# TzuYaoHuang/WaterLily.jl

Measured on AMD Instinct MI355X. Metric: cells*steps/sec (3D TGV) ; smoother HBM GB/s vs peak, higher is better.
Workload: dtype f32; 1 GPU; 3D Taylor-Green vortex 512^3 Float32, wall-bounded, Re=1600, NoBody, remeasure=false (BASELINE configs[4] domain on 1 GPU); size=512, resjac=630, resjac_redo=0

## Files before the change

waterlily.jl_amd/csrc/wl_convf.hip:

```cpp
#include <cstdlib>
#include <type_traits>

#include "wl_bcfold.hpp"
#include "wl_conv_cell.hpp"

namespace {
#define CF_TX 32
#define CF_TY 16
#define CF_N (CF_TX * CF_TY)
#define CF_CX (2 * CF_TX)
#define CF_CY CF_TY
#define CF_W (CF_CX + 4)
#define CF_H (CF_CY + 4)
#define CF_P (CF_W * CF_H)
#define CF_SLOT (3 * CF_P)
#define CF_NSLOT 3
#define CF_HPC (CF_P / 2 - CF_CX / 2 * CF_CY)
#define CF_FYC ((CF_CY + 1) * CF_CX)
#define CF_FY (3 * CF_FYC)
#define CF_FX (3 * CF_CY)
#define CF_FBUF (CF_FY + CF_FX)
#define CF_NGEN (3 * CF_CX + 3 * CF_CY)
#define CF_LDS (CF_NSLOT * CF_SLOT + 2 * CF_FBUF)

struct __attribute__((aligned(4))) F2v { float x, y; };
__device__ __forceinline__ float2 cf_ldg2(const float* __restrict__ p, unsigned o) { const F2v t = *reinterpret_cast<const F2v*>(p + o); return make_float2(t.x, t.y); }
__device__ __forceinline__ void cf_stg2(float* __restrict__ p, unsigned o, float2 v) { F2v t; t.x = v.x; t.y = v.y; *reinterpret_cast<F2v*>(p + o) = t; }
__device__ __forceinline__ float2 cf_lds2(const float* p) { return *reinterpret_cast<const float2*>(p); }
__device__ __forceinline__ float cf_sel(const float2& v, int e) { return e ? v.y : v.x; }
__device__ __forceinline__ float cf_next_lane(float v) {
  return __int_as_float(__builtin_amdgcn_update_dpp(__float_as_int(v), __float_as_int(v), 0x130 , 0xf, 0xf, false));
}

struct CfPair { unsigned off; int mode; };
__device__ __forceinline__ CfPair cf_pair_addr(int X, int Y, int nx, int ny, unsigned sy) {
  CfPair r;
  const int Yc = Y < 0 ? 0 : (Y > ny - 1 ? ny - 1 : Y);
  int Xc = X, mode = 0;
  if (X < 0) { Xc = X + 1; mode = 1; }
  else if (X + 1 > nx - 1) { Xc = X - 1; mode = 2; }
  if (Xc < 0 || Xc + 1 > nx - 1 || Y != Yc) { mode = 3; Xc = Xc < 0 ? 0 : (Xc + 1 > nx - 1 ? nx - 2 : Xc); }
  r.off = (unsigned)Xc + (unsigned)Yc * sy; r.mode = mode;
  return r;
}
__device__ __forceinline__ float2 cf_pair_fix(float2 t, int mode) { return make_float2(mode == 2 ? t.y : t.x, mode == 1 ? t.x : t.y); }

template <int SCH, int WALLS>
__device__ __forceinline__ float cf_flux(float U, float a, float b, float c, float d, bool wl, bool wu, float nu) {
  const bool pos = U > 0;
  float X = lam<SCH>(pos ? a : d, pos ? b : c, pos ? c : b);
  if (WALLS) {
    const bool use_avg = (wl && pos) || (wu && (U < 0));
    X = use_avg ? (c + b) / 2 : X;
  }
  return U * X - nu * (c - b);
}

int g_convf_on = 1;

template <int SCH, int FULL, int U0ADV, int MODE, int PROJ>
__global__ void __launch_bounds__(CF_N, 4) k_conv_flux(GridX g, const float* __restrict__ u, float nu, int ka, int kb, int zchunk, BdimArgs bd) {
  __shared__ float lds[CF_LDS];
  const int ntx = (g.nx - 2 + CF_CX - 1) / CF_CX, nty = (g.ny - 2 + CF_CY - 1) / CF_CY;
  const int ntiles = ntx * nty;
  const unsigned h = blockIdx.x, q = h & 7u, s = h >> 3;
  const unsigned per = (unsigned)((ntiles + 7) >> 3);
  const int c = (int)(s / per);
  const int tl = (int)(q * per + (s - (unsigned)c * per));
  if (tl >= ntiles) return;
  const int ks = ka + c * zchunk, ke = (ks + zchunk < kb) ? ks + zchunk : kb;
  if (ks >= ke) return;
  const int tx = tl % ntx, ty = tl / ntx;
  const int x0 = 1 + tx * CF_CX, y0 = 1 + ty * CF_CY;
  const int tid = threadIdx.x, lx = tid & (CF_TX - 1), ly = tid >> 5;
  const int x = x0 + 2 * lx, y = y0 + ly;
  const int my = (ly + 2) * CF_W + 2 + 2 * lx;
  const bool in0 = FULL || (y <= g.ny - 2 && x <= g.nx - 2), in1 = FULL || (y <= g.ny - 2 && x + 1 <= g.nx - 2);
  const unsigned cs = (unsigned)g.cs, sz = (unsigned)g.sz, sy = (unsigned)g.sy;
  CfPair pc;
  if (FULL) { pc.off = (unsigned)x + (unsigned)y * sy; pc.mode = 0; } else pc = cf_pair_addr(x, y, g.nx, g.ny, sy);
  const int hid = tid < 3 * CF_HPC ? tid : 3 * CF_HPC - 1;
  const int hcmp = hid / CF_HPC, hh = hid - hcmp * CF_HPC;
  int R, col;
  if (hh < 4 * (CF_W / 2)) { const int rr = hh / (CF_W / 2); const int m = hh - rr * (CF_W / 2); R = rr < 2 ? rr : rr + CF_CY; col = 2 * m; }
  else { const int h2 = hh - 4 * (CF_W / 2); R = 2 + (h2 >> 1); col = (h2 & 1) ? CF_W - 2 : 0; }
  const CfPair ph = cf_pair_addr(x0 - 2 + col, y0 - 2 + R, g.nx, g.ny, sy);
  const unsigned hbase = (unsigned)hcmp * cs + ph.off;
  const int hl = hcmp * CF_P + R * CF_W + col;
  const bool gen = tid < CF_NGEN;
  int ga, gF, gsb, gb, gout; bool gwu;
  if (tid < 3 * CF_CX) { ga = tid >> 6; const int gj = tid & 63; gF = (2 + CF_CY) * CF_W + 2 + gj; gsb = CF_W; gb = 1; gwu = (y0 + CF_CY == g.ny - 1); gout = ga * CF_FYC + CF_CY * CF_CX + gj; }
  else { const int t = (tid - 3 * CF_CX) & 63; ga = t >> 4; const int gr = t & 15; gF = (2 + gr) * CF_W + 2 + CF_CX; gsb = 1; gb = 0; gwu = (x0 + CF_CX == g.nx - 1); gout = CF_FY + (ga > 2 ? 2 : ga) * CF_CY + gr; }
  if (ga > 2) ga = 2;
  const int gf = ga * CF_P + gF;
  const int gU0 = gb * CF_P + gF;
  const int gUm = gU0 - (ga == 0 ? 1 : CF_W);
  for (int i = tid; i < CF_LDS; i += CF_N) lds[i] = 0.f;
  __syncthreads();

  struct Stage { float2 c[3]; float2 h; };
  unsigned ho[2] = {0u, 0u}, hnb = 0u; bool hd[2] = {false, false}; float hU = 0.f, hc = 0.f;
  const float* __restrict__ px = bd.px;
  if (PROJ) {
#pragma unroll
    for (int e = 0; e < 2; e++) {
      const int Xe = x0 - 2 + col + e, Ye = y0 - 2 + R;
      const int Xc = Xe < 1 ? 1 : (Xe > g.nx - 2 ? g.nx - 2 : Xe), Yc = Ye < 1 ? 1 : (Ye > g.ny - 2 ? g.ny - 2 : Ye);
      ho[e] = (unsigned)Xc + (unsigned)Yc * sy;
      hd[e] = hcmp == 0 ? (Xe <= 1 || Xe >= g.nx - 1) : (hcmp == 1 ? (Ye <= 1 || Ye >= g.ny - 1) : false);
    }
    hnb = hcmp == 0 ? 1u : (hcmp == 1 ? sy : sz);
    hU = hcmp == 0 ? bd.bcU[0] : (hcmp == 1 ? bd.bcU[1] : bd.bcU[2]);
    hc = hcmp == 0 ? bd.cl_c[0] : (hcmp == 1 ? bd.cl_c[1] : bd.cl_c[2]);
  }
  auto load_plane = [&](int kk) -> Stage {
    const int kc = PROJ ? (kk < 1 ? 1 : (kk > g.nz - 2 ? g.nz - 2 : kk)) : (kk < 0 ? 0 : (kk > g.nz - 1 ? g.nz - 1 : kk));
    const unsigned ko = (unsigned)kc * sz;
    Stage st;
#pragma unroll
    for (int cc = 0; cc < 3; cc++) st.c[cc] = cf_ldg2(u, (unsigned)cc * cs + ko + pc.off);
    if (PROJ) { st.h.x = u[(unsigned)hcmp * cs + ko + ho[0]]; st.h.y = u[(unsigned)hcmp * cs + ko + ho[1]]; }
    else st.h = cf_ldg2(u, hbase + ko);
    return st;
  };
  struct XStage { float2 xc, xy, xk; float xm; float xh[2], xn[2]; };
  auto load_x = [&](int kk) -> XStage {
    const int kc = kk < 1 ? 1 : (kk > g.nz - 2 ? g.nz - 2 : kk);
    const unsigned ko = (unsigned)kc * sz;
    XStage X;
    X.xc = cf_ldg2(px, ko + pc.off); X.xm = px[ko + pc.off - 1u]; X.xy = cf_ldg2(px, ko + pc.off - sy); X.xk = cf_ldg2(px, ko - sz + pc.off);
#pragma unroll
    for (int e = 0; e < 2; e++) { X.xh[e] = px[ko + ho[e]]; X.xn[e] = px[ko + ho[e] - hnb]; }
    return X;
  };
  const bool dxc0 = (x == 1), dyc = (y == 1);
  auto project = [&](Stage& st, const XStage& X, int kk) {
    const bool zd = kk <= 1 || kk >= g.nz - 1;
    const float c0 = bd.cl_c[0], c1 = bd.cl_c[1], c2 = bd.cl_c[2];
    const float p0x = st.c[0].x - c0 * (X.xc.x - X.xm), p0y = st.c[0].y - c0 * (X.xc.y - X.xc.x);
    const float p1x = st.c[1].x - c1 * (X.xc.x - X.xy.x), p1y = st.c[1].y - c1 * (X.xc.y - X.xy.y);
    const float p2x = st.c[2].x - c2 * (X.xc.x - X.xk.x), p2y = st.c[2].y - c2 * (X.xc.y - X.xk.y);
    st.c[0] = make_float2(dxc0 ? bd.bcU[0] : p0x, p0y);
    st.c[1] = make_float2(dyc ? bd.bcU[1] : p1x, dyc ? bd.bcU[1] : p1y);
    st.c[2] = make_float2(zd ? bd.bcU[2] : p2x, zd ? bd.bcU[2] : p2y);
    const float h0 = st.h.x - hc * (X.xh[0] - X.xn[0]), h1 = st.h.y - hc * (X.xh[1] - X.xn[1]);
    const bool hz = hcmp == 2 && zd;
    st.h = make_float2((hd[0] || hz) ? hU : h0, (hd[1] || hz) ? hU : h1);
  };
  auto slot_of = [&](int kk) -> float* { return lds + ((unsigned)(kk + 3) % 3u) * CF_SLOT; };
  auto write_plane = [&](int kk, const Stage& st) {
    float* sl = slot_of(kk);
#pragma unroll
    for (int cc = 0; cc < 3; cc++) *reinterpret_cast<float2*>(sl + cc * CF_P + my) = FULL ? st.c[cc] : cf_pair_fix(st.c[cc], pc.mode);
    *reinterpret_cast<float2*>(sl + hl) = PROJ ? st.h : cf_pair_fix(st.h, ph.mode);
  };
  const bool wlx = (x == 1);
  const bool wux0 = (x == g.nx - 1), wux1 = (x + 1 == g.nx - 1);
  const bool wly = (y == 1), wuy0 = (y == g.ny - 1);
  float zf[3][2];
  float2 Zm1[3];
  float gprev = 0.f;

  auto zfaces = [&](auto ztag, int k, const float2* Zm, const float2* C1, const float2* Zp1, const float2* Zp2, const float* Pp, float (*Pz)[2]) {
    const int Kg = g.gk + k;
    const bool wlz = (Kg + 1 == 1), wuz = (Kg + 1 == g.gnz - 1);
    const float2 Exz = cf_lds2(Pp + 2 * CF_P - 2);
    const float2 Eyz = cf_lds2(Pp + 2 * CF_P - CF_W);
#pragma unroll
    for (int a = 0; a < 3; a++) {
#pragma unroll
      for (int e = 0; e < 2; e++) {
        float Uz;
        if (a == 0) Uz = (cf_sel(Zp1[2], e) + (e ? Zp1[2].x : Exz.y)) / 2;
        else if (a == 1) Uz = (cf_sel(Zp1[2], e) + cf_sel(Eyz, e)) / 2;
        else Uz = (cf_sel(Zp1[2], e) + cf_sel(C1[2], e)) / 2;
        Pz[a][e] = cf_flux<SCH, decltype(ztag)::value>(Uz, cf_sel(Zm[a], e), cf_sel(C1[a], e), cf_sel(Zp1[a], e), cf_sel(Zp2[a], e), wlz, wuz, nu);
      }
    }
  };
  Stage S; XStage XS;
  {
    float2 m2[3];
    if (PROJ) { Stage sm = load_plane(ks - 2); const XStage xm = load_x(ks - 2); project(sm, xm, ks - 2); for (int cc = 0; cc < 3; cc++) m2[cc] = sm.c[cc]; }
    else {
      const unsigned ko = (unsigned)(ks - 2 < 0 ? 0 : ks - 2) * sz;
#pragma unroll
      for (int cc = 0; cc < 3; cc++) { m2[cc] = cf_ldg2(u, (unsigned)cc * cs + ko + pc.off); if (!FULL) m2[cc] = cf_pair_fix(m2[cc], pc.mode); }
    }
    Stage s0 = load_plane(ks - 1), s1 = load_plane(ks), s2 = load_plane(ks + 1);
    if (PROJ) {
      const XStage x0s = load_x(ks - 1), x1s = load_x(ks), x2s = load_x(ks + 1);
      project(s0, x0s, ks - 1); project(s1, x1s, ks); project(s2, x2s, ks + 1);
    }
    S = load_plane(ks + 2);
    if (PROJ) XS = load_x(ks + 2);
    write_plane(ks - 1, s0); write_plane(ks, s1); write_plane(ks + 1, s2);
    float2 C1[3], Zp1[3], Zp2[3];
#pragma unroll
    for (int cc = 0; cc < 3; cc++) {
      C1[cc] = FULL ? s0.c[cc] : cf_pair_fix(s0.c[cc], pc.mode); Zp1[cc] = FULL ? s1.c[cc] : cf_pair_fix(s1.c[cc], pc.mode); Zp2[cc] = FULL ? s2.c[cc] : cf_pair_fix(s2.c[cc], pc.mode);
    }
    __syncthreads();
    zfaces(std::integral_constant<int, 1>{}, ks - 1, m2, C1, Zp1, Zp2, slot_of(ks) + my, zf);
    if (gen) gprev = slot_of(ks - 1)[gU0];
#pragma unroll
    for (int cc = 0; cc < 3; cc++) Zm1[cc] = C1[cc];
    __syncthreads();
  }
  const float dtv = bd.dt_dev ? *bd.dt_dev : bd.dt;
  const int N[3] = {g.nx, g.ny, g.gnz};
  const float mw[2][2] = {{wl::wl_cl_coef(x + 1, N[0], bd.cl_c[0]), wl::wl_cl_coef(x + 2, N[0], bd.cl_c[0])}, {wl::wl_cl_coef(y + 1, N[1], bd.cl_c[1]), wl::wl_cl_coef(y + 1, N[1], bd.cl_c[1])}};
  const bool tile_walls = tx == 0 || tx == ntx - 1 || ty == 0 || ty == nty - 1;
  float2 un[3];
  auto store_plane = [&](auto wtag, int kq) {
    const unsigned kqo = (unsigned)kq * sz;
    if (decltype(wtag)::value && SCH != WL_VANLEER && bd.bc_on && (x <= 1 || x + 1 >= g.nx - 2 || y <= 1 || y >= g.ny - 2)) {
      if (in0) { const float v[3] = {un[0].x, un[1].x, un[2].x}; wl_bc_fold_store_xy(bd.uout, g, x, y, kq, v, bd.bcU); }
      if (in1) { const float v[3] = {un[0].y, un[1].y, un[2].y}; wl_bc_fold_store_xy(bd.uout, g, x + 1, y, kq, v, bd.bcU); }
      return;
    }
#pragma unroll
    for (int a = 0; a < 3; a++) {
      const unsigned oa = (unsigned)a * cs + kqo + pc.off;
      if (FULL) cf_stg2(bd.uout, oa, un[a]);
      else if (pc.mode == 0 && in0 && in1) cf_stg2(bd.uout, oa, un[a]);
      else { const unsigned o0 = (unsigned)a * cs + kqo + (unsigned)x + (unsigned)y * sy; if (in0) bd.uout[o0] = un[a].x; if (in1) bd.uout[o0 + 1] = un[a].y; }
    }
  };
  auto mainloop = [&](auto wtag) {
    constexpr int WALLS = decltype(wtag)::value;
    for (int k = ks; k < ke; k++) {
      if (PROJ) project(S, XS, k + 2);
      float2 Zp2[3];
#pragma unroll
      for (int cc = 0; cc < 3; cc++) Zp2[cc] = FULL ? S.c[cc] : cf_pair_fix(S.c[cc], pc.mode);
      write_plane(k + 2, S);
      S = load_plane(k + 3);
      const unsigned ko = (unsigned)k * sz;
      float2 u0v[3];
      if (k > ks) store_plane(wtag, k - 1);
      const float* S0 = slot_of(k);
      const float* P0 = S0 + my;
      const float* Pp = slot_of(k + 1) + my;
      float* FB = lds + CF_NSLOT * CF_SLOT + (k & 1) * CF_FBUF;
      float2 C1[3], Zp1[3];
#pragma unroll
      for (int cc = 0; cc < 3; cc++) { C1[cc] = cf_lds2(P0 + cc * CF_P); Zp1[cc] = cf_lds2(Pp + cc * CF_P); }
      float a0[3], a1[3], Pl1[3], Px0[3];
      {
        float2 CA[3], Ym2[3], Ym1[3], Yp1[3]; float CCx[3];
#pragma unroll
        for (int cc = 0; cc < 3; cc++) {
          CA[cc] = cf_lds2(P0 + cc * CF_P - 2); CCx[cc] = P0[cc * CF_P + 2];
          Ym2[cc] = cf_lds2(P0 + cc * CF_P - 2 * CF_W); Ym1[cc] = cf_lds2(P0 + cc * CF_P - CF_W); Yp1[cc] = cf_lds2(P0 + cc * CF_P + CF_W);
        }
        const float rx[4] = {CA[0].x, CA[0].y, C1[0].x, C1[0].y};
        const float ry[4] = {CA[1].x, CA[1].y, C1[1].x, C1[1].y};
#pragma unroll
        for (int a = 0; a < 3; a++) {
          const float r[5] = {CA[a].x, CA[a].y, C1[a].x, C1[a].y, CCx[a]};
          float Ux[2];
          if (a == 0) { Ux[0] = (rx[2] + rx[1]) / 2; Ux[1] = (rx[3] + rx[2]) / 2; }
          else if (a == 1) { Ux[0] = (rx[2] + Ym1[0].x) / 2; Ux[1] = (rx[3] + Ym1[0].y) / 2; }
          else { Ux[0] = (rx[2] + Zm1[0].x) / 2; Ux[1] = (rx[3] + Zm1[0].y) / 2; }
          const float PxA = cf_flux<SCH, WALLS>(Ux[0], r[0], r[1], r[2], r[3], wlx, wux0, nu);
          const float PxB = cf_flux<SCH, WALLS>(Ux[1], r[1], r[2], r[3], r[4], false, wux1, nu);
          float t0 = 0.f, t1 = 0.f;
          t0 = t0 + PxA; t0 = t0 - PxB;
          t1 = t1 + PxB;
          Px0[a] = PxA;
          float Pl[2];
#pragma unroll
          for (int e = 0; e < 2; e++) {
            const float vm2 = cf_sel(Ym2[a], e), vm1 = cf_sel(Ym1[a], e), v0 = cf_sel(C1[a], e), vp1 = cf_sel(Yp1[a], e);
            float Ul;
            if (a == 0) Ul = (ry[2 + e] + ry[1 + e]) / 2;
            else if (a == 1) Ul = (v0 + vm1) / 2;
            else Ul = (cf_sel(C1[1], e) + cf_sel(Zm1[1], e)) / 2;
            Pl[e] = cf_flux<SCH, WALLS>(Ul, vm2, vm1, v0, vp1, wly, wuy0, nu);
          }
          t0 = t0 + Pl[0];
          a0[a] = t0; a1[a] = t1; Pl1[a] = Pl[1];
          *reinterpret_cast<float2*>(FB + a * CF_FYC + ly * CF_CX + 2 * lx) = make_float2(Pl[0], Pl[1]);
        }
      }
      if (gen) {
        const float fa = S0[gf - 2 * gsb], fb = S0[gf - gsb], fc = S0[gf], fd = S0[gf + gsb];
        const float ub0 = S0[gU0], ubm = S0[gUm];
        const float U = (ub0 + (ga == 2 ? gprev : ubm)) / 2;
        gprev = ub0;
        FB[gout] = cf_flux<SCH, WALLS>(U, fa, fb, fc, fd, false, gwu, nu);
      }
      float Pz[3][2];
      const int Kg = g.gk + k;
      const bool zwall = (Kg + 1 == 1 || Kg + 1 == g.gnz - 1);
      if (zwall) zfaces(std::integral_constant<int, 1>{}, k, Zm1, C1, Zp1, Zp2, Pp, Pz);
      else zfaces(std::integral_constant<int, 0>{}, k, Zm1, C1, Zp1, Zp2, Pp, Pz);
      if (!U0ADV) {
#pragma unroll
        for (int a = 0; a < 3; a++) { u0v[a] = cf_ldg2(bd.u0, (unsigned)a * cs + ko + pc.off); if (!FULL) u0v[a] = cf_pair_fix(u0v[a], pc.mode); }
      }
      if (PROJ) XS = load_x(k + 3);
      __syncthreads();
      float2 PuA[3]; float PxE[3];
#pragma unroll
      for (int a = 0; a < 3; a++) {
        PuA[a] = cf_lds2(FB + a * CF_FYC + (ly + 1) * CF_CX + 2 * lx);
        PxE[a] = 0.f;
        if (lx == CF_TX - 1) PxE[a] = FB[CF_FY + a * CF_CY + ly];
      }
      const float mz = wl::wl_cl_coef(Kg + 1, N[2], bd.cl_c[2]);
#pragma unroll
      for (int a = 0; a < 3; a++) {
        float Px2 = cf_next_lane(Px0[a]);
        if (lx == CF_TX - 1) Px2 = PxE[a];
        const float2 Pu = PuA[a];
        float t0 = a0[a], t1 = a1[a];
        t0 = t0 - Pu.x;
        t1 = t1 - Px2; t1 = t1 + Pl1[a]; t1 = t1 - Pu.y;
        t0 = t0 + zf[a][0]; t0 = t0 - Pz[a][0]; zf[a][0] = Pz[a][0];
        t1 = t1 + zf[a][1]; t1 = t1 - Pz[a][1]; zf[a][1] = Pz[a][1];
        const float acc[2] = {t0, t1};
        const float2 u0a = U0ADV ? C1[a] : u0v[a];
        const float m00 = a == 2 ? mz : (WALLS ? mw[a][0] : bd.cl_c[a]), m01 = a == 2 ? mz : (WALLS ? mw[a][1] : bd.cl_c[a]);
#pragma unroll
        for (int e = 0; e < 2; e++) {
          const float fn = cf_sel(u0a, e) + dtv * acc[e] - 0.f;
          const float xx = (0.f / 2 + 0.f) + (e ? m01 : m00) * fn;
          float v;
          if (MODE == 1) v = xx;
          else if (MODE == 2) v = (cf_sel(C1[a], e) * bd.pre + xx) * bd.post;
          else { v = (bd.pre == 0.f) ? xx : (cf_sel(C1[a], e) * bd.pre + xx); if (bd.scale_after) v = v * bd.post; }
          if (e) un[a].y = v; else un[a].x = v;
        }
        Zm1[a] = C1[a];
      }
    }
    store_plane(wtag, ke - 1);
  };
  if (tile_walls) mainloop(std::integral_constant<int, 1>{}); else mainloop(std::integral_constant<int, 0>{});
}
}

namespace wl {
void conv_flux_enable(int on) { g_convf_on = on; }
bool conv_flux_on() { return g_convf_on != 0; }
bool conv_proj_ok(const GridX& g, unsigned per) {
  return g_convf_on && g.D == 3 && g.nz == g.gnz && g.k0 == 1 && g.k1 == g.nz - 1 && g.nz >= 6 && (g.nx - 2) % CF_CX == 0 && (g.ny - 2) % CF_CY == 0 && conv_tile_ok(g, per, g.k1 - g.k0);
}
int conv_flux(const float* u_adv, const GridX& g, float nu, int scheme, int ka, int kb, int zc, const void* bdp, hipStream_t s) {
  const BdimArgs bd = *(const BdimArgs*)bdp;
  const int ntiles = ((g.nx - 2 + CF_CX - 1) / CF_CX) * ((g.ny - 2 + CF_CY - 1) / CF_CY);
  const int per = (ntiles + 7) >> 3;
  const int np = kb - ka;
  const int nch = (np + zc - 1) / zc;
  const dim3 grid((unsigned)(8 * per * nch), 1, 1);
  const bool full = (g.nx - 2) % CF_CX == 0 && (g.ny - 2) % CF_CY == 0;
  const bool u0adv = bd.u0 == u_adv;
  const int mode = (u0adv && bd.pre == 0.f && !bd.scale_after) ? 1 : ((!u0adv && bd.pre != 0.f && bd.scale_after) ? 2 : 0);
  if (bd.px && !(full && mode == 2 && g.nz == g.gnz && ka == 1 && kb == g.nz - 1)) { wl_set_error("conv_flux: the fused projection needs whole tiles, the corrector's BDIM! form and the whole single domain"); return WL_EINVAL; }
#define WL_CF(SCHV, FULLV, ADV, MD, PJ) hipLaunchKernelGGL((k_conv_flux<SCHV, FULLV, ADV, MD, PJ>), grid, dim3(CF_N), 0, s, g, u_adv, nu, ka, kb, zc, bd)
#define WL_CF1(SCHV, FULLV) do { if (mode == 1) WL_CF(SCHV, FULLV, 1, 1, 0); else if (mode == 2) WL_CF(SCHV, FULLV, 0, 2, 0); else if (u0adv) WL_CF(SCHV, FULLV, 1, 0, 0); else WL_CF(SCHV, FULLV, 0, 0, 0); } while (0)
#define WL_CF2(SCHV) do { if (bd.px) WL_CF(SCHV, 1, 0, 2, 1); else if (full) WL_CF1(SCHV, 1); else WL_CF1(SCHV, 0); } while (0)
  switch (scheme) {
    case WL_QUICK: WL_CF2(WL_QUICK); break;
    case WL_VANLEER: WL_CF2(WL_VANLEER); break;
    case WL_CDS: WL_CF2(WL_CDS); break;
    default: wl_set_error("unknown scheme"); return WL_EINVAL;
  }
#undef WL_CF2
#undef WL_CF1
#undef WL_CF
  WL_LAUNCH_CHECK(); return 0;
}
}
```

waterlily.jl_amd/csrc/wl_sim.hip:

```cpp
#include <cmath>
#include <cstring>
#include <utility>
#include <vector>

#include "wl_common.hpp"
#include <algorithm>
#include "wl_mg.hpp"
#include "wl_body.hpp"
#include "wl_pdefer.hpp"

namespace {
__device__ __forceinline__ bool cell_ij(const GridX& g, long m, int& i, int& j) {
  if (m >= g.sz) return false;
  j = (int)(m / g.nx);
  i = (int)(m - (long)j * g.nx);
  return true;
}
__device__ __forceinline__ bool interior_ij(const GridX& g, int i, int j) { return i >= 1 && i <= g.nx - 2 && j >= 1 && j <= g.ny - 2; }

template <int D>
__global__ void k_apply_tgv(GridX g, float* __restrict__ u, float kx, float ky, float kz) {
  int i, j; long m; int pz;
  wl_tile(g, m, pz);
  if (!cell_ij(g, m, i, j)) return;
// ... 184 lines not shown
template <int D>
__global__ void k_exit_update_slab(GridX g, float* __restrict__ u, const float* __restrict__ u0, const double* __restrict__ sc, float dt, int mode) {
  const int ny = g.ny - 2;
  const long cnt = (long)ny * (g.k1 - g.k0);
  const long q = (long)blockIdx.x * WL_BLOCK + threadIdx.x;
  if (q >= cnt) return;
  const int j = 1 + (int)(q % ny), k = g.k0 + (int)(q / ny);
  const long o = (g.nx - 1) + (long)j * g.sy + (long)k * g.sz;
  if (mode == 0) { const float U = (float)sc[0]; u[o] = u0[o] - U * dt * (u0[o] - u0[o - 1]); }
  else u[o] -= (float)sc[1];
}
__global__ void k_dt_from_cfl(float* __restrict__ res_f, int in_slot, int out_slot, float nu) { res_f[out_slot] = fminf(10.f, 1.0f / (res_f[in_slot] + 5 * nu)); }
template <int D>
__global__ void k_exit_update(GridX g, float* __restrict__ u, const float* __restrict__ u0, const double* __restrict__ sc, float dt, int mode) {
  const int ny = g.ny - 2;
  const long cnt = (long)ny * ((D == 3) ? (g.nz - 2) : 1);
  const long q = (long)blockIdx.x * WL_BLOCK + threadIdx.x;
  if (q >= cnt) return;
  const int j = 1 + (int)(q % ny), k = (D == 3) ? 1 + (int)(q / ny) : 0;
  const long o = (g.nx - 1) + (long)j * g.sy + (long)k * g.sz;
  if (mode == 0) { const float U = (float)sc[0]; u[o] = u0[o] - U * dt * (u0[o] - u0[o - 1]); }
  else u[o] -= (float)sc[1];
}
}

#define DSEL(D, KERN, ...)                                                           \
  do { if ((D) == 3) hipLaunchKernelGGL(KERN<3>, __VA_ARGS__); else hipLaunchKernelGGL(KERN<2>, __VA_ARGS__); } while (0)

struct wl_sim {
  wl_sim_desc d;
  wl_grid g; GridX G;
  float *u = nullptr, *u0 = nullptr, *f = nullptr, *p = nullptr, *sigma = nullptr, *V = nullptr, *mu0 = nullptr, *mu1 = nullptr;
  float* own = nullptr;
  wl_mg* mg = nullptr;
  wl_comm* comm = nullptr;
  bool swap_ok = false;
  float* ps = nullptr;
  bool use_fuse_p = true;
  double* exit_sc = nullptr;
  bool forcing = false;
  float acc0[3] = {0, 0, 0}, acc1[3] = {0, 0, 0};
  float* us = nullptr;
  int sgs_model = 0;
  float sgs_Cs = 0.f, sgs_Delta = 1.f;
  int sgs_udf(const float* uadv, hipStream_t s) { return sgs_model ? wl::sgs(f, sigma, uadv, G, sgs_Cs, sgs_Delta, s) : 0; }
  std::vector<float> dt;
  bool own_mg = true;
  ~wl_sim() { if (u_pending && comm && comm->cs) (void)hipStreamSynchronize(comm->cs); if (own_mg) delete mg; if (own) (void)hipFree(own); if (exit_sc) (void)hipFree(exit_sc); if (farmask) (void)hipFree(farmask); if (mnear) (void)hipFree(mnear); if (mneedf) (void)hipFree(mneedf); if (mm0var) (void)hipFree(mm0var); }

  bool use_overlap = true;
  bool u_pending = false;
  int sync_u(hipStream_t s) { if (u_pending) { u_pending = false; return wl::halo_async_wait(comm, s); } return 0; }
  int use_bcfold = 1; bool bc_folded = false;
  bool fold_ok(int bit) const { return (use_bcfold & bit) && d.D == 3 && !comm && !d.exitBC && !d.perdir_mask && G.nz == G.gnz && G.nx >= 6 && G.ny >= 6 && G.nz >= 6; }
  BcFold fold_req(int bit) const { BcFold f{fold_ok(bit) ? 1 : 0, {d.uBC[0], d.uBC[1], d.uBC[2]}}; return f; }
  int bc_u(hipStream_t s) {
    WL_TRY(sync_u(s));
    if (bc_folded) { bc_folded = false; return 0; }
    WL_TRY(wl::bc_vec(u, G, d.uBC, d.exitBC, d.perdir_mask, s));
    if (comm && use_overlap) { WL_TRY(wl::halo_async_begin(comm, u, G, d.D, 2, s)); u_pending = true; return 0; }
    return wl::halo(comm, u, G, d.D, 2, s);
  }
  bool store_f = false;
  int conv_fused(const float* uadv, float* uout, float pre, float post, hipStream_t s, bool want_q1 = true, const float* dt_dev = nullptr) {
    const wl::ConstL& cl = mg->lv[0].cl;
    float* f = store_f ? this->f : nullptr;
    if (u_pending && G.D == 3 && G.k1 - G.k0 > 4) {
      if (dt_dev) { wl_set_error("conv_fused: Δt on the device is for the single domain"); return WL_EINVAL; }
      WL_TRY(wl::conv_diff_bdim(f, uadv, sigma, u0, mu0, uout, G, d.nu, d.perdir_mask, d.scheme, dt.back(), pre, post, cl, s, G.k0 + 2, G.k1 - 2, false));
      WL_TRY(sync_u(s));
      WL_TRY(wl::conv_diff_bdim(f, uadv, sigma, u0, mu0, uout, G, d.nu, d.perdir_mask, d.scheme, dt.back(), pre, post, cl, s, -(1 << 30), G.k0 + 2, false));
      return wl::conv_diff_bdim(f, uadv, sigma, u0, mu0, uout, G, d.nu, d.perdir_mask, d.scheme, dt.back(), pre, post, cl, s, G.k1 - 2, 1 << 30, want_q1);
    }
    WL_TRY(sync_u(s));
    BcFold fr = fold_req(2);
    fr.proj_x = proj_pending;
    fr.dt_dev = dt_dev;
    WL_TRY(wl::conv_diff_bdim(f, uadv, sigma, u0, mu0, uout, G, d.nu, d.perdir_mask, d.scheme, dt.back(), pre, post, cl, s, -(1 << 30), 1 << 30, want_q1, &fr));
    if (proj_pending && !fr.proj_done) { wl_set_error("mom_step!: the corrector did not take the deferred projection"); return WL_EINVAL; }
    proj_pending = nullptr;
    bc_folded = fr.on != 0;
    return 0;
  }
  bool use_tailfuse = false;
  const float* proj_pending = nullptr;
  bool tailfuse_ok() const {
    return use_tailfuse && fold_ok(3) && us && !d.has_body && !forcing && !sgs_model && !store_f && !use_convz && !u_pending && mg->lv[0].cl.on && !mg->lv[0].part &&
           wl::conv_proj_ok(G, d.perdir_mask);
  }
  bool use_convz = false;
  int conv_only(const float* uadv, hipStream_t s) {
    WL_TRY(sync_u(s));
    if (use_convz && wl::conv_z_ok(G, d.perdir_mask)) {
      WL_TRY(wl::conv_diff_z(f, uadv, nullptr, nullptr, nullptr, G, d.nu, d.scheme, 0.f, 0.f, 1.f, s));
      return wl::conv_q1(sigma, uadv, G, d.nu, d.perdir_mask, d.scheme, s);
    }
    return wl::conv_diff(f, uadv, sigma, G, d.nu, d.perdir_mask, d.scheme, s);
  }
  unsigned char* farmask = nullptr;
  bool use_farmask = true, mask_valid = false;
  unsigned char *mnear = nullptr, *mneedf = nullptr, *mm0var = nullptr;
  int near_box[4] = {0, -1, 0, -1};
  int dirty_z[2] = {0, -1};
  bool use_hybrid = true;
  bool hybrid_ok() const { return d.has_body && use_hybrid && mask_valid && mnear && us && !comm && !forcing && !sgs_model && !d.exitBC; }
  int refresh_body_mask(hipStream_t s) {
    if (!d.has_body || !mu1 || !V) return 0;
    if (!farmask) WL_HIP(hipMalloc((void**)&farmask, wl::body_mask_bytes(G)));
    if (!mnear) { const size_t nb = (size_t)wl::body_masks_nbm(G) * (size_t)G.nz; WL_HIP(hipMalloc((void**)&mnear, nb)); WL_HIP(hipMalloc((void**)&mneedf, nb)); WL_HIP(hipMalloc((void**)&mm0var, nb)); }
    mask_valid = true;
    WL_TRY(wl::body_masks(mnear, mneedf, mm0var, V, mu1, mu0, G, s));
    WL_TRY(wl::body_masks_box(mnear, G, near_box, s));
    WL_TRY(wl::body_masks_planes(mnear, mneedf, mm0var, G, dirty_z, s));
    return wl::body_mask(farmask, V, mu1, G, s);
  }
  int conv_bdim_body(const float* uadv, float* uout, float pre, float post, hipStream_t s) {
    WL_TRY(sync_u(s));
    { ProfScope pc(WL_PROF_CONVDIFF, s);
      WL_TRY(wl::conv_diff_bdim_body(f, uadv, sigma, u0, mu0, uout, G, d.nu, d.perdir_mask, d.scheme, dt.back(), pre, post, mnear, mneedf, mm0var, wl::body_masks_nbm(G), store_f ? 1 : 0, s, dirty_z[0], dirty_z[1])); }
    ProfScope pb(WL_PROF_BDIM, s);
    return wl::bdim_near(uout, u, u0, f, V, mu0, mu1, G, dt.back(), pre, post, mnear, wl::body_masks_nbm(G), near_box, s);
  }
  int bdim_step(float pre, float post, hipStream_t s) {
    ProfScope pb(WL_PROF_BDIM, s);
    if (d.has_body) {
      WL_TRY(wl::bdim_f(f, u0, V, G, dt.back(), s));
      if (comm) WL_TRY(wl::halo(comm, f, G, d.D, 1, s));
      return wl::bdim_u(u, f, V, mu0, mu1, G, pre, post, s, (use_farmask && mask_valid) ? farmask : nullptr);
    }
    return wl::bdim(u, u0, f, nullptr, mu0, nullptr, G, dt.back(), pre, post, s);
  }
  int exit_bc(hipStream_t s);
  int copy_exit_face(float* dst, const float* src, hipStream_t s);
  bool use_bcdefer = true, in_step = false, bc_deferred = false;
  long n_bcdefer = 0;
  bool head_fused_ok() const {
    const wl_mg::Level& l0 = mg->lv[0];
    return ps && use_fuse_p && use_resjac && !resjac_backoff && (!resjac_force_redo || redo_unannounced) && !d.exitBC && !store_f && !d.perdir_mask && !l0.part && mg->defer_shift && mg->lv.size() > 1 &&
           wl::resjac_ok(G, l0.cl) && !comm;
  }
  bool bcdefer_ok(bool second) const {
    if (!(use_bcdefer && in_step && !bc_folded && fold_ok(1) && head_fused_ok())) return false;
    return !second || (use_fuse_cfl && us && wl::project_cfl_pair_path(G, mg->lv[0].cl));
  }
  int bc_u_or_defer(bool second, hipStream_t s) {
    if (bcdefer_ok(second)) { bc_deferred = true; n_bcdefer++; return 0; }
    return bc_u(s);
  }
  int flush_bc(hipStream_t s) {
    if (!bc_deferred) return 0;
    bc_deferred = false;
    return wl::bc_vec(u, G, d.uBC, d.exitBC, d.perdir_mask, s);
  }
  int predict(hipStream_t s, const float* dt_dev = nullptr) {
    if (hybrid_ok()) {
      WL_TRY(conv_bdim_body(u0, u, 0.f, 1.f, s));
      return bc_u(s);
    }
    bool fused_conv = false;
    if (us && !d.has_body && !forcing && !sgs_model) {
      ProfScope pc(WL_PROF_CONVDIFF, s);
      if (use_convz && wl::conv_z_ok(G, d.perdir_mask)) {
        WL_TRY(sync_u(s));
        WL_TRY(wl::conv_diff_z(store_f ? f : nullptr, u0, u0, mu0, u, G, d.nu, d.scheme, dt.back(), 0.f, 1.f, s));
        WL_TRY(wl::conv_q1(sigma, u0, G, d.nu, d.perdir_mask, d.scheme, s));
      } else { WL_TRY(conv_fused(u0, u, 0.f, 1.f, s, !(in_step && !store_f), dt_dev)); fused_conv = true; }
    } else {
      { ProfScope pc(WL_PROF_CONVDIFF, s); WL_TRY(conv_only(u0, s)); }
      WL_TRY(sgs_udf(u0, s));
      if (forcing) WL_TRY(wl::accelerate(f, G, acc0, s));
      WL_TRY(bdim_step(0.f, 1.f, s));
// ... 376 lines not shown
  if (trials > 1) {
    size_t fr = 0, tot = 0;
    if (hipMemGetInfo(&fr, &tot) == hipSuccess) { const long fit = (long)(fr / 2 / ((size_t)cells * 160 + 1)); if (fit < trials) trials = fit < 1 ? 1 : (int)fit; }
  }
  g_last_placement_n = 0;
  if (trials == 1) return sim_create_common(out, desc, nullptr);
  wl_sim* cand[8] = {nullptr}; double score[8]; int best = -1;
  for (int i = 0; i < trials; i++) {
    const int rc = sim_create_common(&cand[i], desc, nullptr);
    if (rc != 0) { cand[i] = nullptr; if (best < 0 && i == trials - 1) return rc; break; }
    score[i] = placement_score(cand[i]);
    g_last_placement[g_last_placement_n++] = score[i];
    if (best < 0 || score[i] < score[best]) best = i;
  }
  if (best < 0) return WL_EINVAL;
  for (int i = 0; i < trials; i++) if (cand[i] && i != best) delete cand[i];
  *out = cand[best];
  return 0;
}
int wl_placement_scores(double* out, int cap) { int k = 0; for (; k < g_last_placement_n && k < cap; k++) out[k] = g_last_placement[k]; return g_last_placement_n; }
int wl_sim_create_on(wl_sim** out, const wl_sim_desc* desc, wl_mg* mg) { WL_CHECK(mg, "null wl_mg"); return sim_create_common(out, desc, nullptr, mg); }
int wl_sim_create_slab(wl_sim** out, const wl_sim_desc* desc, wl_comm* comm) { return sim_create_common(out, desc, comm); }
int wl_sim_destroy(wl_sim* s) { delete s; return 0; }
float* wl_sim_field(wl_sim* s, const char* name) {
  const std::string n(name);
  (void)s->sync_u(0);
  if (n == "p") (void)s->materialise_p(0);
  if (n == "V" || n == "mu1" || n == "mu0") s->mask_valid = false;
  if (n == "u") return s->u; if (n == "u0") return s->u0; if (n == "f") return s->f; if (n == "p") { if (s->p_shell != 2) s->p_shell = -1; return s->p; }
  if (n == "sigma") return s->sigma; if (n == "V") return s->V; if (n == "mu0") return s->mu0; if (n == "mu1") return s->mu1;
  if (n == "us") return s->us;
  return nullptr;
}
wl_mg* wl_sim_pois(wl_sim* s) { return s->mg; }
int wl_sim_grid(const wl_sim* s, wl_grid* out) { *out = s->g; return 0; }
int wl_sim_init_flow(wl_sim* s, void* st) {
  hipStream_t q = wl_stream(st);
  WL_TRY(s->bc_u(q));
  if (s->d.exitBC) {
    const float keep = s->dt.back(); float* keep0 = s->u0;
    s->dt.back() = 0.f; s->u0 = s->u;
    const int rc = s->exit_bc(q);
    s->dt.back() = keep; s->u0 = keep0;
    if (rc != 0) return rc;
  }
  WL_HIP(hipMemcpyAsync(s->u0, s->u, sizeof(float) * (size_t)s->G.cs * s->d.D, hipMemcpyDeviceToDevice, q));
  return 0;
}
int wl_sim_set_option(wl_sim* s, const char* name, int value) {
  const std::string n(name);
  if (n == "convz") { s->use_convz = value != 0; return 0; }
  if (n == "fused_smoother") { s->mg->use_fused = value != 0; return 0; }
  if (n == "store_eps") { s->mg->store_eps = value != 0; return 0; }
  if (n == "constl") { s->mg->use_constl = value != 0; return s->mg->update(0); }
  if (n == "tail") { s->mg->use_tail = value != 0; return 0; }
  if (n == "tail_lds") { wl::tail_lds_enable(value); return 0; }
  if (n == "xdefer") { s->mg->use_xdefer = value != 0; return 0; }
  if (n == "overlap_smooth") { s->mg->overlap_smooth = value != 0; return 0; }
  if (n == "body_tile") { wl::conv_body_tile_enable(value); return 0; }
  if (n == "skip_fill") { s->mg->skip_fill = value != 0; return 0; }
  if (n == "defer_shift") { s->mg->defer_shift = value != 0; return 0; }
  if (n == "zsplit") {
    s->mg->use_zsplit = value != 0; s->mg->zsplit_min = value == 2 ? 0 : (value >= 4 ? (long)value << 20 : 16L << 20); return 0;
  }
  if (n == "hybrid") { s->use_hybrid = value != 0; return 0; }
  if (n == "farmask") { s->use_farmask = value != 0; return 0; }
  if (n == "store_f") { s->store_f = value != 0; return 0; }
  if (n == "overlap") { WL_TRY(s->sync_u(0)); s->use_overlap = value != 0; return 0; }
  if (n == "fuse_cfl") { s->use_fuse_cfl = value != 0; return 0; }
  if (n == "jacobi_march") { wl::jacobi_march_enable(value); return 0; }
  if (n == "convm") { wl::conv_march_enable(value); return 0; }
  if (n == "deep_halo") { s->mg->deep_halo = value != 0; return 0; }
  if (n == "x_halo") { if (value < 1 || value > s->G.k0) { wl_set_error("x_halo: 1 .. ghost depth of the slab"); return WL_EINVAL; } s->mg->x_halo_depth = value; return 0; }
  if (n == "bcfold") { s->use_bcfold = value; return 0; }
  if (n == "resjac") { s->use_resjac = value != 0; s->resjac_force_redo = value == 2 || value == 3; s->redo_unannounced = value == 3; return 0; }
  if (n == "resjac_min") { wl::resjac_enable(1, value); return 0; }
  if (n == "convt_min") { wl::conv_tile_min(value); return 0; }
  if (n == "lazydt") { s->use_lazydt = value != 0; return 0; }
  if (n == "tailspec") { s->use_tailspec = value != 0; return 0; }
  if (n == "headspec") { s->use_headspec = value != 0; return 0; }
  if (n == "bcdefer") { s->use_bcdefer = value != 0; return 0; }
  if (n == "pdefer") { s->use_pdefer = value != 0; return 0; }
  if (n == "tailwide") { s->use_tailwide = value != 0; return 0; }
  if (n == "tailfuse") { s->use_tailfuse = value != 0; return 0; }
  if (n == "convf") { wl::conv_flux_enable(value != 0); return 0; }
  if (n == "convt") { wl::conv_tile_enable(value != 0, value > 1 ? value : 0); return 0; }
  if (n == "pair") { wl::gsrb_pair_enable(value); return 0; }
  if (n == "fuse_p") { s->use_fuse_p = value != 0; return 0; }
  if (n == "zsplit_par") { s->mg->par_ranges = value != 0; return 0; }
  if (n == "itmx") { if (value < 1) { wl_set_error("itmx must be >= 1"); return WL_EINVAL; } s->itmx = value; return 0; }
  wl_set_error("unknown option " + n); return WL_EINVAL;
}
int wl_sim_update(wl_sim* s, void* st) { s->resjac_backoff = false; s->resjac_redo_run = 0; WL_TRY(s->refresh_body_mask(wl_stream(st))); return s->mg->update(wl_stream(st)); }

long wl_launch_count(void) { return g_wl_launches; }
int wl_reset_process_options(void) {
  wl::resjac_enable(1, 6L << 20); wl::conv_tile_min(2048); wl::conv_tile_enable(1, 0); wl::conv_flux_enable(1); wl::tail_lds_enable(1); wl::conv_body_tile_enable(1);
  wl::gsrb_pair_enable(1); wl::jacobi_march_enable(1); wl::conv_march_enable(0);
  return 0;
}
int wl_sim_counter(wl_sim* s, const char* name, long* out) {
  WL_CHECK(s && name && out, "bad argument");
  const std::string n(name);
  if (n == "resjac") { *out = s->n_resjac; return 0; }
  if (n == "resjac_redo") { *out = s->n_resjac_redo; return 0; }
  if (n == "resjac_backoff") { *out = s->resjac_backoff ? 1 : 0; return 0; }
  if (n == "tailfuse") { *out = s->n_tailfuse; return 0; }
  if (n == "bcdefer") { *out = s->n_bcdefer; return 0; }
  if (n == "pdefer") { *out = s->n_pdefer; return 0; }
  if (n == "tailwide") { *out = s->n_tailwide; return 0; }
  if (n == "tailspec") { *out = s->n_tailspec; return 0; }
  if (n == "tailspec_armed") { *out = s->n_tailspec_armed; return 0; }
  if (n == "xdefer") { *out = s->mg->last_xdefer; return 0; }
  wl_set_error("unknown counter " + n); return WL_EINVAL;
}
int wl_sim_set_forcing(wl_sim* s, const float* U1, const float* a0, const float* a1) {
  const int D = s->d.D;
  if (U1) for (int c = 0; c < D; c++) s->d.uBC[c] = U1[c];
  s->forcing = a0 != nullptr || a1 != nullptr;
  for (int c = 0; c < 3; c++) { s->acc0[c] = (a0 && c < D) ? a0[c] : 0.f; s->acc1[c] = (a1 && c < D) ? a1[c] : 0.f; }
  return 0;
}
int wl_sim_set_sgs(wl_sim* s, int model, float Cs, float Delta) {
  WL_CHECK(s, "null wl_sim"); WL_CHECK(model == 0 || model == 1, "wl_sim_set_sgs: model must be 0 (off) or 1 (Smagorinsky-Lilly)");
  if (model) {
    if (s->d.D != 3) { wl_set_error("wl_sim_set_sgs: the Smagorinsky model is built for 3-D flows only"); return WL_EINVAL; }
    if (s->comm) { wl_set_error("wl_sim_set_sgs: z-slab handles are not supported (single domain only)"); return WL_EINVAL; }
  }
  s->sgs_model = model; s->sgs_Cs = Cs; s->sgs_Delta = Delta;
  return 0;
}
int wl_accelerate(float* r, const wl_grid* g, const float* a, void* st) {
  WL_CHECK(wl_grid_ok(g) && a, "bad argument"); WL_TRY(wl_ctx_ensure());
  return wl::accelerate(r, gx(*g), a, wl_stream(st));
}
int wl_sim_mom_step(wl_sim* s, void* st) { return s->mom_step(wl_stream(st)); }
int wl_sim_mom_steps(wl_sim* s, int n, void* st) {
  WL_CHECK(s && n >= 0, "bad argument");
  for (int k = 0; k < n; k++) WL_TRY(s->mom_step(wl_stream(st), k + 1 < n));
  return 0;
}
int wl_sim_dt(const wl_sim* s, float* out, int cap) { const int n = (int)s->dt.size(); for (int k = 0; k < n && k < cap; k++) out[k] = s->dt[(size_t)k]; return n; }
float wl_sim_dt_last(const wl_sim* s) { return s->dt.back(); }
int wl_sim_set_dt_last(wl_sim* s, float dt) { WL_CHECK(s && dt > 0.f, "bad Δt"); s->dt.back() = dt; return 0; }
double wl_sim_time(const wl_sim* s) { float t = 0.f; for (size_t k = 0; k + 1 < s->dt.size(); k++) t += s->dt[k]; return (double)t; }
int wl_sim_phase(wl_sim* s, int phase, void* st) {
  hipStream_t q = wl_stream(st);
  WL_TRY(s->materialise_p(q));
  switch (phase) {
    case 0: WL_TRY(s->sync_u(q)); WL_HIP(hipMemcpyAsync(s->u0, s->u, sizeof(float) * (size_t)s->G.cs * s->d.D, hipMemcpyDeviceToDevice, q)); return wl::scale_u(s->u, s->G, 0.f, q);
    case 1: return s->predict(q);
    case 2: return s->project(1.f, q);
    case 3: return s->correct(q);
    case 4: return s->project(0.5f, q);
    case 5: return s->cfl(q);
  }
  wl_set_error("bad phase"); return WL_EINVAL;
}
int wl_sim_apply_ic(wl_sim* s, int kind, void* st) {
  hipStream_t q = wl_stream(st); const GridX& G = s->G; const int D = s->d.D;
  if (kind == 0) { DSEL(D, k_apply_const, wl_plane_grid(G, G.nz), dim3(WL_BLOCK), 0, q, G, s->u, s->d.uBC[0], s->d.uBC[1], s->d.uBC[2]); }
  else {
    const float two = (kind == 2) ? 2.f : 1.f;
    const float kx = two * 3.14159265358979323846f / (float)s->d.dims[0], ky = two * 3.14159265358979323846f / (float)s->d.dims[1];
    const float kz = (D == 3) ? two * 3.14159265358979323846f / (float)s->d.dims[2] : 0.f;
    DSEL(D, k_apply_tgv, wl_plane_grid(G, G.nz), dim3(WL_BLOCK), 0, q, G, s->u, kx, ky, kz);
  }
  WL_LAUNCH_CHECK(); return 0;
}
static int to_body_arg(int D, const wl_body* b, BodyArg* o) {
  WL_CHECK(b && (b->kind == WL_BODY_SPHERE || b->kind == WL_BODY_PLANE), "wl_body.kind must be WL_BODY_SPHERE or WL_BODY_PLANE");
  o->kind = b->kind; o->R = b->R;
  float mm = 0.f;
  for (int q = 0; q < 3; q++) { o->c[q] = q < D ? b->c[q] : 0.f; o->m[q] = q < D ? b->m[q] : 0.f; o->V[q] = q < D ? b->V[q] : 0.f; mm += o->m[q] * o->m[q]; }
  WL_CHECK(mm > 0.f, "wl_body.m (axis mask / plane normal) is zero");
  return 0;
}
static wl_body sphere_body(const float* c, float R) {
  wl_body b{}; b.kind = WL_BODY_SPHERE; b.R = R;
  for (int q = 0; q < 3; q++) { b.c[q] = c[q]; b.m[q] = 1.f; }
  return b;
}
static int measure_fields(float* sigma, float* mu0, float* mu1, float* V, const GridX& G, const BodyArg& bd, float eps, int exitBC, unsigned perdir, hipStream_t q) {
  const int D = G.D; const size_t nc = (size_t)G.cs;
  WL_TRY(wl::fill(V, 0.f, nc * D, q)); WL_TRY(wl::fill(mu0, 1.f, nc * D, q)); WL_TRY(wl::fill(mu1, 0.f, nc * D * D, q));
  DSEL(D, k_measure_body, wl_plane_grid(G, G.k1 - G.k0), dim3(WL_BLOCK), 0, q, G, sigma, mu0, mu1, V, bd, eps);
  WL_LAUNCH_CHECK();
  const float zero[3] = {0, 0, 0};
  WL_TRY(wl::bc_vec(mu0, G, zero, 0, perdir, q));
  return wl::bc_vec(V, G, zero, exitBC, perdir, q);
// ... 110 lines not shown
```

Baseline: 14.77 billion cells*steps/s.

## Enable fused projection tail in conv-flux kernel with leaner register staging

Turns on the tailfuse path by default for large domains (above a cell-count threshold), so the pressure projection is folded into the convection-flux kernel. The projected plane's loads are restructured to cut register pressure: the z-neighbour of the potential is carried over from the previous plane, the x-neighbour is fetched with a cross-lane DPP shift instead of a global load, and the generator-thread flux indices are parked in LDS. The projection of the next plane is moved after the flux generation so that fewer values stay live at once. In exchange it uses more LDS per block and adds dependence on lane ordering, and a new size gate decides whether the fused path runs.

```diff
diff --git a/waterlily.jl_amd/csrc/wl_convf.hip b/waterlily.jl_amd/csrc/wl_convf.hip
--- a/waterlily.jl_amd/csrc/wl_convf.hip
+++ b/waterlily.jl_amd/csrc/wl_convf.hip
@@ -22,6 +22,7 @@
 #define CF_FBUF (CF_FY + CF_FX)
 #define CF_NGEN (3 * CF_CX + 3 * CF_CY)
 #define CF_LDS (CF_NSLOT * CF_SLOT + 2 * CF_FBUF)
+#define CF_GENC 5
 
 struct __attribute__((aligned(4))) F2v { float x, y; };
 __device__ __forceinline__ float2 cf_ldg2(const float* __restrict__ p, unsigned o) { const F2v t = *reinterpret_cast<const F2v*>(p + o); return make_float2(t.x, t.y); }
@@ -30,6 +31,9 @@
 __device__ __forceinline__ float cf_sel(const float2& v, int e) { return e ? v.y : v.x; }
 __device__ __forceinline__ float cf_next_lane(float v) {
   return __int_as_float(__builtin_amdgcn_update_dpp(__float_as_int(v), __float_as_int(v), 0x130 , 0xf, 0xf, false));
+}
+__device__ __forceinline__ float cf_prev_lane(float v) {
+  return __int_as_float(__builtin_amdgcn_update_dpp(__float_as_int(v), __float_as_int(v), 0x138 , 0xf, 0xf, false));
 }
 
 struct CfPair { unsigned off; int mode; };
@@ -60,7 +64,7 @@
 
 template <int SCH, int FULL, int U0ADV, int MODE, int PROJ>
 __global__ void __launch_bounds__(CF_N, 4) k_conv_flux(GridX g, const float* __restrict__ u, float nu, int ka, int kb, int zchunk, BdimArgs bd) {
-  __shared__ float lds[CF_LDS];
+  __shared__ float lds[CF_LDS + (PROJ ? CF_GENC * 256 : 0)];
   const int ntx = (g.nx - 2 + CF_CX - 1) / CF_CX, nty = (g.ny - 2 + CF_CY - 1) / CF_CY;
   const int ntiles = ntx * nty;
   const unsigned h = blockIdx.x, q = h & 7u, s = h >> 3;
@@ -96,6 +100,8 @@
   const int gU0 = gb * CF_P + gF;
   const int gUm = gU0 - (ga == 0 ? 1 : CF_W);
   for (int i = tid; i < CF_LDS; i += CF_N) lds[i] = 0.f;
+  int* const genc = reinterpret_cast<int*>(lds + CF_LDS) + (tid & 255);
+  if (PROJ && gen) { genc[0] = gf; genc[256] = gsb; genc[512] = gU0; genc[768] = gUm; genc[1024] = gout; }
   __syncthreads();
 
   struct Stage { float2 c[3]; float2 h; };
@@ -129,6 +135,18 @@
     const unsigned ko = (unsigned)kc * sz;
     XStage X;
     X.xc = cf_ldg2(px, ko + pc.off); X.xm = px[ko + pc.off - 1u]; X.xy = cf_ldg2(px, ko + pc.off - sy); X.xk = cf_ldg2(px, ko - sz + pc.off);
+#pragma unroll
+    for (int e = 0; e < 2; e++) { X.xh[e] = px[ko + ho[e]]; X.xn[e] = px[ko + ho[e] - hnb]; }
+    return X;
+  };
+  struct XLean { float2 xc, xy; float xm; float xh[2], xn[2]; };
+  float2 xkp = make_float2(0.f, 0.f);
+  auto load_x_lean = [&](int kk) -> XLean {
+    const int kc = kk < 1 ? 1 : (kk > g.nz - 2 ? g.nz - 2 : kk);
+    const unsigned ko = (unsigned)kc * sz;
+    XLean X;
+    X.xc = cf_ldg2(px, ko + pc.off); X.xy = cf_ldg2(px, ko + pc.off - sy);
+    X.xm = 0.f; if (lx == 0) X.xm = px[ko + pc.off - 1u];
 #pragma unroll
     for (int e = 0; e < 2; e++) { X.xh[e] = px[ko + ho[e]]; X.xn[e] = px[ko + ho[e] - hnb]; }
     return X;
@@ -147,6 +165,16 @@
     const bool hz = hcmp == 2 && zd;
     st.h = make_float2((hd[0] || hz) ? hU : h0, (hd[1] || hz) ? hU : h1);
   };
+  auto project_lean = [&](Stage& st, const XLean& L, int kk) {
+    XStage X;
+    X.xc = L.xc; X.xy = L.xy; X.xk = xkp;
+    const float pm = cf_prev_lane(L.xc.y);
+    X.xm = lx == 0 ? L.xm : pm;
+#pragma unroll
+    for (int e = 0; e < 2; e++) { X.xh[e] = L.xh[e]; X.xn[e] = L.xn[e]; }
+    project(st, X, kk);
+    xkp = L.xc;
+  };
   auto slot_of = [&](int kk) -> float* { return lds + ((unsigned)(kk + 3) % 3u) * CF_SLOT; };
   auto write_plane = [&](int kk, const Stage& st) {
     float* sl = slot_of(kk);
@@ -178,7 +206,7 @@
       }
     }
   };
-  Stage S; XStage XS;
+  Stage S;
   {
     float2 m2[3];
     if (PROJ) { Stage sm = load_plane(ks - 2); const XStage xm = load_x(ks - 2); project(sm, xm, ks - 2); for (int cc = 0; cc < 3; cc++) m2[cc] = sm.c[cc]; }
@@ -191,9 +219,9 @@
     if (PROJ) {
       const XStage x0s = load_x(ks - 1), x1s = load_x(ks), x2s = load_x(ks + 1);
       project(s0, x0s, ks - 1); project(s1, x1s, ks); project(s2, x2s, ks + 1);
+      xkp = x2s.xc;
     }
     S = load_plane(ks + 2);
-    if (PROJ) XS = load_x(ks + 2);
     write_plane(ks - 1, s0); write_plane(ks, s1); write_plane(ks + 1, s2);
     float2 C1[3], Zp1[3], Zp2[3];
 #pragma unroll
@@ -230,12 +258,15 @@
   auto mainloop = [&](auto wtag) {
     constexpr int WALLS = decltype(wtag)::value;
     for (int k = ks; k < ke; k++) {
-      if (PROJ) project(S, XS, k + 2);
       float2 Zp2[3];
-#pragma unroll
-      for (int cc = 0; cc < 3; cc++) Zp2[cc] = FULL ? S.c[cc] : cf_pair_fix(S.c[cc], pc.mode);
-      write_plane(k + 2, S);
-      S = load_plane(k + 3);
+      XLean XL;
+      if (PROJ) XL = load_x_lean(k + 2);
+      else {
+#pragma unroll
+        for (int cc = 0; cc < 3; cc++) Zp2[cc] = FULL ? S.c[cc] : cf_pair_fix(S.c[cc], pc.mode);
+        write_plane(k + 2, S);
+        S = load_plane(k + 3);
+      }
       const unsigned ko = (unsigned)k * sz;
       float2 u0v[3];
       if (k > ks) store_plane(wtag, k - 1);
@@ -285,11 +316,19 @@
         }
       }
       if (gen) {
-        const float fa = S0[gf - 2 * gsb], fb = S0[gf - gsb], fc = S0[gf], fd = S0[gf + gsb];
-        const float ub0 = S0[gU0], ubm = S0[gUm];
+        const int qf = PROJ ? genc[0] : gf, qsb = PROJ ? genc[256] : gsb, qU0 = PROJ ? genc[512] : gU0, qUm = PROJ ? genc[768] : gUm, qout = PROJ ? genc[1024] : gout;
+        const float fa = S0[qf - 2 * qsb], fb = S0[qf - qsb], fc = S0[qf], fd = S0[qf + qsb];
+        const float ub0 = S0[qU0], ubm = S0[qUm];
         const float U = (ub0 + (ga == 2 ? gprev : ubm)) / 2;
         gprev = ub0;
-        FB[gout] = cf_flux<SCH, WALLS>(U, fa, fb, fc, fd, false, gwu, nu);
+        FB[qout] = cf_flux<SCH, WALLS>(U, fa, fb, fc, fd, false, gwu, nu);
+      }
+      if (PROJ) {
+        project_lean(S, XL, k + 2);
+#pragma unroll
+        for (int cc = 0; cc < 3; cc++) Zp2[cc] = S.c[cc];
+        write_plane(k + 2, S);
+        S = load_plane(k + 3);
       }
       float Pz[3][2];
       const int Kg = g.gk + k;
@@ -300,7 +339,6 @@
 #pragma unroll
         for (int a = 0; a < 3; a++) { u0v[a] = cf_ldg2(bd.u0, (unsigned)a * cs + ko + pc.off); if (!FULL) u0v[a] = cf_pair_fix(u0v[a], pc.mode); }
       }
-      if (PROJ) XS = load_x(k + 3);
       __syncthreads();
       float2 PuA[3]; float PxE[3];
 #pragma unroll
diff --git a/waterlily.jl_amd/csrc/wl_sim.hip b/waterlily.jl_amd/csrc/wl_sim.hip
--- a/waterlily.jl_amd/csrc/wl_sim.hip
+++ b/waterlily.jl_amd/csrc/wl_sim.hip
@@ -290,11 +290,13 @@
     bc_folded = fr.on != 0;
     return 0;
   }
-  bool use_tailfuse = false;
+  static constexpr long TAILFUSE_MIN_DEFAULT = 16L << 20;
+  bool use_tailfuse = true;
+  long tailfuse_min = TAILFUSE_MIN_DEFAULT;
   const float* proj_pending = nullptr;
   bool tailfuse_ok() const {
     return use_tailfuse && fold_ok(3) && us && !d.has_body && !forcing && !sgs_model && !store_f && !use_convz && !u_pending && mg->lv[0].cl.on && !mg->lv[0].part &&
-           wl::conv_proj_ok(G, d.perdir_mask);
+           (long)(G.nx - 2) * (G.ny - 2) * (G.gnz - 2) >= tailfuse_min && wl::conv_proj_ok(G, d.perdir_mask);
   }
   bool use_convz = false;
   int conv_only(const float* uadv, hipStream_t s) {
@@ -837,7 +839,8 @@
   if (n == "bcdefer") { s->use_bcdefer = value != 0; return 0; }
   if (n == "pdefer") { s->use_pdefer = value != 0; return 0; }
   if (n == "tailwide") { s->use_tailwide = value != 0; return 0; }
-  if (n == "tailfuse") { s->use_tailfuse = value != 0; return 0; }
+  if (n == "tailfuse") { s->use_tailfuse = value != 0; if (value != 0) s->tailfuse_min = 0; return 0; }
+  if (n == "tailfuse_min") { if (value < 0) { wl_set_error("tailfuse_min: interior cells, >= 0"); return WL_EINVAL; } s->tailfuse_min = value; return 0; }
   if (n == "convf") { wl::conv_flux_enable(value != 0); return 0; }
   if (n == "convt") { wl::conv_tile_enable(value != 0, value > 1 ? value : 0); return 0; }
   if (n == "pair") { wl::gsrb_pair_enable(value); return 0; }
@@ -861,6 +864,7 @@
   if (n == "resjac_redo") { *out = s->n_resjac_redo; return 0; }
   if (n == "resjac_backoff") { *out = s->resjac_backoff ? 1 : 0; return 0; }
   if (n == "tailfuse") { *out = s->n_tailfuse; return 0; }
+  if (n == "tailfuse_min") { *out = s->tailfuse_min; return 0; }
   if (n == "bcdefer") { *out = s->n_bcdefer; return 0; }
   if (n == "pdefer") { *out = s->n_pdefer; return 0; }
   if (n == "tailwide") { *out = s->n_tailwide; return 0; }
```

Measured after the change: 15.77 billion cells*steps/s, median of 6. 1.07x the previous value.
